# BEAMRobotics/beam_slam

Hardware: AMD Instinct MI355X
Metric: LM iterations/sec + ms/graph-solve, 200KF x 50k-landmark VIO window (higher is better)
Workload: dtype f64; 1 GPU; C2: 200-keyframe x 50000-landmark VIO window; n_obs=400690, n_imu_factors=199, solver_options=vio.yaml:7-17 (<= 10 iterations, tolerances 1.5e-7), max_solver_time lifted, parallelism=single GPU, n_ranks_seen=1

## Files before the change

beam_slam_amd/csrc/band_plan.h:

```cpp
#pragma once
#include <cstdint>
#include <vector>

#include "bsgpu_internal.h"

namespace bsg {

__host__ __device__ inline bool band_record(int b, int e, const int* cam_pose, int* cmin, int4* rec) {
  *cmin = -1;
  *rec = make_int4(0, 0, -1, -1);
  if (e - b < 2 || e - b > kBandCams) return false;
  int lo = cam_pose[b], hi = cam_pose[b];
  for (int f = b + 1; f < e; ++f) { lo = cam_pose[f] < lo ? cam_pose[f] : lo; hi = cam_pose[f] > hi ? cam_pose[f] : hi; }
  if (hi - lo >= kBandCams) return false;
  unsigned m = 0;
  uint64_t inv = ~(uint64_t)0;
  for (int f = b; f < e; ++f) {
    const int sl = cam_pose[f] - lo;
    const unsigned bit = 1u << sl;
    if (m & bit) return false;
    m |= bit;
    inv = (inv & ~((uint64_t)15 << (4 * sl))) | ((uint64_t)(f - b) << (4 * sl));
  }
  *cmin = lo;
  *rec = make_int4(b, (int)(m | ((unsigned)(hi - lo + 1) << 16) | ((unsigned)(e - b) << 24)), (int)(uint32_t)inv, (int)(uint32_t)(inv >> 32));
  return true;
}

inline void band_classify_host(int nl, const int* lm_start, const int* cam_pose, std::vector<int>& cmin, std::vector<int>& mask, std::vector<int4>& rec) {
  cmin.assign(nl, -1); mask.assign(nl, 0);
  rec.assign(nl, make_int4(0, 0, -1, -1));
  for (int l = 0; l < nl; ++l)
    if (band_record(lm_start[l], lm_start[l + 1], cam_pose, &cmin[l], &rec[l])) mask[l] = rec[l].y & 0xffff;
}

struct BandUnits {
  std::vector<int> lm;
  std::vector<int> unit_start, unit_cam;
  std::vector<uint32_t> adj;
};

int band_part_forced();

inline void band_units(int nl, const int* cmin, const int* mask, int ncp, BandUnits& out) {
  out.lm.clear(); out.unit_start.clear(); out.unit_cam.clear();
  const size_t nc = (size_t)(ncp > 0 ? ncp : 1);
  out.adj.assign(nc, 0);
  const size_t nkey = nc * 16;
  std::vector<int> start(nkey + 1, 0);
  auto span_of = [&](int l) { int top = 0; for (unsigned m = (unsigned)mask[l]; m; m >>= 1) ++top; return top; };
  auto key_of = [&](int l) { return (size_t)cmin[l] * 16 + (size_t)(kBandCams - span_of(l)); };
  int n = 0;
  for (int l = 0; l < nl; ++l) if (cmin[l] >= 0) { start[key_of(l) + 1]++; ++n; }
  out.unit_start.push_back(0);
  if (!n) return;
  for (size_t k = 0; k < nkey; ++k) start[k + 1] += start[k];
  out.lm.resize(n);
  for (int l = 0; l < nl; ++l) if (cmin[l] >= 0) out.lm[start[key_of(l)]++] = l;
  out.unit_start.clear();
  int part = band_part_forced();
  if (part <= 0) part = n / 128 > 64 ? n / 128 : 64;
  std::vector<std::vector<unsigned>> seen(nc);
  int i = 0;
  while (i < n) {
    const int k0 = cmin[out.lm[i]];
    int j = i;
    while (j < n && cmin[out.lm[j]] == k0) {
      const unsigned m = (unsigned)mask[out.lm[j]];
      bool have = false;
      for (unsigned s : seen[k0]) if (s == m) { have = true; break; }
      if (!have) {
        seen[k0].push_back(m);
        for (int a = 0; a < kBandCams; ++a)
          if ((m >> a) & 1u) out.adj[k0 + a] |= (m >> a);
      }
      ++j;
    }
    const int parts = (j - i + part - 1) / part;
    for (int p = 0; p < parts; ++p) { out.unit_start.push_back(i + (int)((int64_t)(j - i) * p / parts)); out.unit_cam.push_back(k0); }
    i = j;
  }
  out.unit_start.push_back(n);
}

}
```

beam_slam_amd/csrc/bsgpu_finalize.cpp:

```cpp
#include <atomic>

#include "bsgpu_ctx.h"
#include "bsgpu_env.h"
#include "band_plan.h"
#include "dim_order.h"

namespace bsg {

int band_part_forced() {
  return env_int("BSGPU_BAND_PART", 0);
}

namespace {
void eigen_quat_to_rot(const double* q, double* R) {
  const double tx = 2 * q[1], ty = 2 * q[2], tz = 2 * q[3];
  const double twx = tx * q[0], twy = ty * q[0], twz = tz * q[0], txx = tx * q[1], txy = ty * q[1], txz = tz * q[1];
  const double tyy = ty * q[2], tyz = tz * q[2], tzz = tz * q[3];
  R[0] = 1 - (tyy + tzz); R[1] = txy - twz; R[2] = txz + twy;
  R[3] = txy + twz; R[4] = 1 - (txx + tzz); R[5] = tyz - twx;
  R[6] = txz - twy; R[7] = tyz + twx; R[8] = 1 - (txx + tyy);
}

}

int finalize(bsgpu_ctx* c) {
  if (c->finalized) return BSGPU_OK;
  const bool timing = env_timing();
  auto t_prev = std::chrono::steady_clock::now();
  auto lap = [&](const char* what) {
    if (!timing) return;
    const auto now = std::chrono::steady_clock::now();
    fprintf(stderr, "[bsgpu finalize] %-28s %8.2f ms\n", what, std::chrono::duration<double, std::milli>(now - t_prev).count());
    t_prev = now;
  };
  c->free_device();
  HIPCHK(c, hipSetDevice(c->device));
  lap("free previous");
  const int nb = c->nb;
  if (nb <= 0) return fail(c, BSGPU_ERR_INVALID, "no parameter blocks");
  std::vector<int> lm_use(nb, 0), other_use(nb, 0), rho_use(nb, 0);
  for (int t = 0; t < BSGPU_F_NUM_TYPES; ++t) {
    const HostGroup& g = c->groups[t];
    const TypeInfo& ti = kTypes[t];
    if (t == BSGPU_F_REPROJ && c->mirror0.active && !c->mirror0.materialized) {
      const SlotMirror& m = c->mirror0;
      const size_t ns = std::max({m.use_q.size(), m.use_p.size(), m.use_l.size()});
// ... 256 lines not shown
      cp_keys.erase(std::unique(cp_keys.begin(), cp_keys.end()), cp_keys.end());
    }
    const int k = (int)cp_keys.size();
    std::vector<int> cp_tq, cp_tp, cp_first(nb, -1);
    for (int i = 0; i < k; ++i) {
      const int bq = (int)(cp_keys[i] >> 32), bp = (int)(cp_keys[i] & 0xffffffffu);
      cp_tq.push_back(c->toff[bq]); cp_tp.push_back(c->toff[bp]);
      if (cp_first[bq] < 0) cp_first[bq] = i;
    }
    auto cp_of = [&](int bq, int bp) {
      int i = cp_first[bq];
      while ((int)(cp_keys[i] & 0xffffffffu) != bp) ++i;
      return i;
    };
    V.n_cam_pose = k;
    int n_elim = 0;
    for (int i = 0; i < nv; ++i) {
      const VF& e = vf[i];
      fac[i] = make_int4(e.xq, e.xp, e.xl, meta_pack(e.meta_cam, e.loss, e.flags));
      pix[i] = make_double2(e.u, e.v);
      w[i] = e.w;
      cam_pose[i] = cp_of(e.bq, e.bp);
      lm_of[i] = e.lm;
      c->vis_src[i] = e.src;
      if (e.lm >= 0) { lm_start[e.lm + 1]++; n_elim++; }
    }
    for (int l = 0; l < nl; ++l) lm_start[l + 1] += lm_start[l];
    V.n_elim = n_elim;
    lap("camera-pose ids");
    std::vector<int> b_cmin(nl, -1), b_mask(nl, 0);
    std::vector<int4> b_rec;
    if (band_on && nl > 0) band_classify_host(nl, lm_start.data(), cam_pose.data(), b_cmin, b_mask, b_rec);
    BandUnits bu;
    band_units(nl, b_cmin.data(), b_mask.data(), V.n_cam_pose, bu);
    std::vector<int4> b_lm(bu.lm.size());
    for (size_t i = 0; i < bu.lm.size(); ++i) b_lm[i] = b_rec[bu.lm[i]];
    V.n_band_lm = (int)bu.lm.size(); V.n_band_units = (int)bu.unit_cam.size();
    lap("band landmarks");
    const uint64_t ncp = (uint64_t)std::max(1, V.n_cam_pose);
    std::vector<int> seg_ci, seg_cj, seg_start, ent_fa, ent_fb;
    if (ncp * ncp <= (uint64_t)8 << 20 && !sort_entries) {
      std::vector<int> start(ncp * ncp + 1, 0);
      for (int l = 0; l < nl; ++l) {
        if (b_cmin[l] >= 0) continue;
        for (int a = lm_start[l]; a < lm_start[l + 1]; ++a) {
          const uint64_t ra = (uint64_t)cam_pose[a] * ncp;
          for (int b = lm_start[l]; b < lm_start[l + 1]; ++b) if (cam_pose[a] <= cam_pose[b]) start[ra + cam_pose[b] + 1]++;
        }
      }
      for (int f = n_elim; f < nv; ++f) start[(uint64_t)cam_pose[f] * ncp + cam_pose[f] + 1]++;
      for (size_t i = 0; i < ncp * ncp; ++i) start[i + 1] += start[i];
      const size_t n_ent = (size_t)start[ncp * ncp];
      ent_fa.resize(n_ent); ent_fb.resize(n_ent);
      lap("count pair entries");
      const int chunk = pair_chunk(n_ent);
      for (uint64_t key = 0; key < ncp * ncp; ++key)
        for (int p0 = start[key]; p0 < start[key + 1]; p0 += chunk) { seg_ci.push_back((int)(key / ncp)); seg_cj.push_back((int)(key % ncp)); seg_start.push_back(p0); }
      std::vector<int> pos(start.begin(), start.end() - 1);
      for (int l = 0; l < nl; ++l) {
        if (b_cmin[l] >= 0) continue;
        for (int a = lm_start[l]; a < lm_start[l + 1]; ++a) {
          const uint64_t ra = (uint64_t)cam_pose[a] * ncp;
          for (int b = lm_start[l]; b < lm_start[l + 1]; ++b)
            if (cam_pose[a] <= cam_pose[b]) { const int p = pos[ra + cam_pose[b]]++; ent_fa[p] = a; ent_fb[p] = b; }
        }
      }
      for (int f = n_elim; f < nv; ++f) { const int p = pos[(uint64_t)cam_pose[f] * ncp + cam_pose[f]]++; ent_fa[p] = f; ent_fb[p] = f; }
      lap("fill pair entries");
    } else {
      struct Ent { uint64_t key; int fa, fb; };
// ... 74 lines not shown
      cb.seg_cp = c->upload(sg_cp); cb.seg_start = c->upload(sg_start); cb.seg_fac = c->upload(by_cp);
      const int re[2] = {cb.tq, cb.tp};
      for (int a = 0; a < 2; ++a) {
        for (int b = 0; b < 2; ++b) touch(re[a], re[b]);
        for (int i = 0; i < k; ++i) { touch(cp_tq[i], re[a]); touch(cp_tp[i], re[a]); }
      }
    }
  }
    return BSGPU_OK;
  };
  bool flattened_on_device = false;
  {
    const bool force_dev = env_flatten_is("device"), force_host = env_flatten_is("host");
    const HostGroup& g0 = c->groups[BSGPU_F_REPROJ];
    SlotMirror& mir = c->mirror0;
    const bool resident = mir.active && !mir.materialized && mir.dev_valid;
    if (!force_host && c->groups[BSGPU_F_REPROJ_ONLINE_CALIB].n == 0 && g0.n > 0 && (force_dev || g0.n >= kDeviceFlattenMin)) {
      bool ok = true;
      if (mir.active && !mir.materialized && !resident) { const int rc_m = materialize_mirror(c); if (rc_m != BSGPU_OK) return rc_m; }
      if (resident) { for (const auto& u : mir.loss_use) if (u.rows > 0 && ok) { get_loss(u.kind, u.a); ok = losses.size() <= 8; } }
      else for (int f = 0; f < g0.n && ok; ++f) { get_loss(g0.loss_kind[f], g0.loss_a[f]); ok = losses.size() <= 8; }
      if (ok) {
        std::vector<int> bx(c->off.begin(), c->off.end());
        std::vector<unsigned char> bc(c->is_const.begin(), c->is_const.end());
        const int* d_bx = c->upload(bx); const int* d_bt = c->upload(c->toff);
        const unsigned char* d_bc = c->upload(bc); const int* d_bl = c->upload(lm_index);
        const int T = (c->n_pose + 63) / 64;
        bool all_const = false;
        FlattenSegsHost segs_host;
        auto dalloc = [&](size_t bytes) -> void* { return c->alloc<unsigned char>(bytes); };
        const FlattenResident res = {mir.d_idx, mir.d_consts, mir.d_lk, mir.d_la, mir.d_s2b};
        const int st = flatten_visual_device(c->stream, dalloc, g0.n, g0.idx.data(), g0.consts.data(), g0.loss_kind.data(), g0.loss_a.data(),
                                             losses, nb, d_bx, d_bt, d_bc, d_bl, nl, T, c->vis, &c->d_vis_src, c->tile_adj, &all_const,
                                             resident ? &res : nullptr, bg.nbk ? &segs_host : nullptr, band_on);
        if (st < 0) return fail(c, BSGPU_ERR_DEVICE, "device error while flattening the reprojection factors");
        if (st == 0) {
          flattened_on_device = true;
          if (bg.nbk)
            for (size_t sgi = 0; sgi < segs_host.seg_ci.size(); ++sgi) {
              const int i = segs_host.seg_ci[sgi], j = segs_host.seg_cj[sgi];
              const int ri[2] = {segs_host.cp_tq[i], segs_host.cp_tp[i]}, rj[2] = {segs_host.cp_tq[j], segs_host.cp_tp[j]};
              for (int a = 0; a < 2; ++a) for (int b = 0; b < 2; ++b) if (ri[a] >= 0 && rj[b] >= 0) bg.add(ri[a], rj[b]);
            }
          if (all_const) { c->any_inactive = true; c->vis_any_inactive = true; }
          if (c->vis.n_cam_pose >= (1 << 20)) return fail(c, BSGPU_ERR_UNSUPPORTED, "too many camera poses");
        } else {
          c->vis = Visual();
        }
      }
    }
  }
  if (flattened_on_device) lap("flatten on device");
  else { const int rc_host = host_visual(); if (rc_host != BSGPU_OK) return rc_host; }
  Visual& V = c->vis;
  {
    const int nv = V.n;
    V.r = c->alloc<double2>(nv); V.J = c->alloc<double>((size_t)nv * (kJAStride + 6)); V.JB = V.J ? V.J + (size_t)nv * kJAStride : nullptr; V.CR = c->alloc<double>((size_t)nv * 8);
    V.Linv = c->alloc<double>((size_t)std::max(1, nl) * kLmRec); V.z = V.Linv ? V.Linv + 6 : nullptr;
    V.n_cost_part = (nv + 255) / 256;
    V.cost_part = c->alloc<double>(V.n_cost_part);
    V.cost_part_cand = c->alloc<double>(V.n_cost_part);
    V.mcc_part = c->alloc<double>(std::max(1, backsub_mcc_groups(V)));
    if (!V.J || !V.CR || !V.r) return fail(c, BSGPU_ERR_DEVICE, "out of device memory (visual tables)");
    if (c->calib.on) {
      c->calib.E = c->alloc<double>((size_t)std::max(1, nv) * 12); c->calib.Et = c->alloc<double>((size_t)std::max(1, nv) * 12);
      c->calib.part = c->alloc<double>((size_t)std::max(1, calib_border_blocks(V)) * kCalibPartStride);
      if (!c->calib.E || !c->calib.Et || !c->calib.part) return fail(c, BSGPU_ERR_DEVICE, "out of device memory (extrinsic border tables)");
// ... 868 lines not shown
```

beam_slam_amd/csrc/bsgpu_internal.h:

```cpp
#pragma once
#include <hip/hip_runtime.h>
#include <stdint.h>

#include <functional>
#include <cstring>
#include <vector>

#include "dense_plan.h"

struct bsgpu_options;

namespace bsg {

struct DevCamera {
  double fx, fy, cx, cy;
  double R[9];
  double t[3];
};
struct DevLoss {
  int kind;
  int pad;
  double a;
};

// ... 429 lines not shown
                               int bridge_gap, double min_excitation, int apply_scale, double scale_min, double scale_max, double rank_tol,
                               double* gravity, double* bg, double* scale, double* excitation, int* gyro_rank, double* velocity,
                               double* q_out, double* p_out, double* v_out, int* status, int* own, double* fs, double* ps);
void launch_triangulate(hipStream_t s, int n_tracks, const int* track_start, const int2* pose_off, const double2* pix, const double* x,
                        const DevCamera& cam, bool truncate, double max_dist, double max_reproj, double* points, int* status);
constexpr int kLocOutStride = 45;
void launch_localize(hipStream_t s, int n_frames, const int* obs_start, const double2* pix, const double* pts, const int* pt_off,
                     const double* x, const DevCamera* cams, const int* cam_of, const double* pose_in, int loss_kind, double loss_a,
                     double sqrt_info, int truncate, int min_points, int width, int height, const bsgpu_options& opt, double* out,
                     int* out_i);
constexpr int kRansacOutInts = 8;
void launch_essential_ransac(hipStream_t s, int n_sets, const int* match_start, const double2* px_prev, const double2* px_cur,
                             const double* K, double prob, double threshold_px, int max_iters, uint64_t seed, unsigned char* mask,
                             double* out_E, int* out_i);
constexpr int kP3pOutDoubles = 19;
constexpr int kP3pOutInts = 6;
void launch_absolute_pose_ransac(hipStream_t s, int n_frames, const int* obs_start, const double2* pix, const double* pts,
                                 const DevCamera* cams, const int* cam_of, double prob, double threshold_px, int max_iters, uint64_t seed,
                                 int truncate, unsigned char* mask, double* out_d, int* out_i);
constexpr int kRelposeOutDoubles = 27;
constexpr int kRelposeOutInts = 11;
void launch_relative_pose_ransac(hipStream_t s, int n_sets, const int* match_start, const double2* pix_first, const double2* pix_last,
                                 const DevCamera* cams, const int* cam_of, double prob, double threshold_px, int max_iters, uint64_t seed,
                                 int truncate, double validate_px, double min_inlier_ratio, unsigned char* mask, unsigned char* valid_mask,
                                 double* points, double* out_d, int* out_i);
struct FlattenResident { const int* idx; const double* consts; const int* loss_kind; const double* loss_a; const int* slot_map; };
struct FlattenSegsHost { std::vector<int> seg_ci, seg_cj, cp_tq, cp_tp; };
void launch_patch_factor_rows(hipStream_t s, int n_ch, const int* rows, const int* idx4, const double* consts3, const int* lk, const double* la,
                              int* dst_idx, double* dst_consts, int* dst_lk, double* dst_la);
int flatten_visual_device(hipStream_t s, const std::function<void*(size_t)>& dalloc, int n, const int* h_idx, const double* h_consts,
                          const int* h_loss_kind, const double* h_loss_a, const std::vector<DevLoss>& losses, int nb, const int* d_blk_xoff,
                          const int* d_blk_toff, const unsigned char* d_blk_const, const int* d_blk_lm, int nl, int T, Visual& V,
                          int** d_vis_src, std::vector<unsigned char>& tile_adj, bool* any_all_const, const FlattenResident* res = nullptr,
                          FlattenSegsHost* segs_out = nullptr, bool band_enabled = true);
int chol_vinv_stride();
void chol_prepare();
void launch_bsr_assemble(hipStream_t s, const SmallGroup& g, const int* slots, double* val);
void launch_bsr_assemble_seg(hipStream_t s, const SmallGroup* groups_dev, int n_seg, const int* seg_start, const int* seg_slot, const int* seg_row,
                             const int2* contrib, double* val, double* rhs, double* grad, double* hdiag);
void launch_bsr_finish_diag(hipStream_t s, int nbr, const int* diag_slot, const int* pair_slot, double* val, const double* hdiag, double radius,
                            int compute_scale, int compute_dcl, int jacobi, double lm_lo, double lm_hi, double* scale,
                            double* dcl, double* Minv);
int pcg_spmv_grid(int nbr);
struct PcgPersistDev {
  int G = 0, max_cols = 0;
  int paired = 0;
  const int *wg_row = nullptr, *wg_colptr = nullptr, *wg_cols = nullptr, *lcol = nullptr;
  unsigned long long* slots = nullptr;
  int* abort_w = nullptr;
  double* zg = nullptr;
  size_t sync_bytes = 0;
  int n_coarse = 0;
  const int4* co = nullptr;
  double centre[3] = {0.0, 0.0, 0.0};
  double *W = nullptr, *E = nullptr, *Einv = nullptr;
  unsigned* counter = nullptr;
};
size_t pcg_coarse_scratch_doubles(int nbr);
void launch_pcg_coarse(hipStream_t s, const PcgPersistDev& P, int nbr, const int* row_ptr, const int* col, const double* val, const double* x);
size_t pcg_persistent_lds(int max_cols);
size_t pcg_persistent_lds_limit();
int pcg_persistent_max_rows();
size_t pcg_persistent_slot_words(int G);
size_t pcg_persistent_z_words(int nbr);
bool launch_pcg_persistent(hipStream_t s, const PcgPersistDev& P, int nbr, const int* row_ptr, const double* val, const double* Minv, const double* b,
                           double* x, double* zg, double* sc, double tol2, int max_it);
void launch_pcg_init(hipStream_t s, int nbr, const double* b, const double* Minv, double* x, double* r, double* z, double* p0, double* p1,
// ... 50 lines not shown
```

beam_slam_amd/csrc/k_flatten.hip:

```cpp
#include <string.h>

#include <cstring>

#include <rocprim/rocprim.hpp>

#include <cstdint>
#include <functional>
#include <vector>

#include "bsgpu_device.h"
#include "band_plan.h"

namespace bsg {

namespace {

__global__ void fl_prep_kernel(int n, const int* __restrict__ idx , const double* __restrict__ consts ,
                               const int* __restrict__ loss_kind, const double* __restrict__ loss_a, int n_loss,
                               const int* __restrict__ tab_kind, const double* __restrict__ tab_a, const int* __restrict__ blk_xoff,
                               const unsigned char* __restrict__ blk_const, const int* __restrict__ blk_lm, int nl,
                               unsigned* __restrict__ key, int4* __restrict__ fac, double2* __restrict__ pix, double* __restrict__ w,
                               int* __restrict__ lm_of, int* __restrict__ bq_of, int* __restrict__ used_q, int* __restrict__ p_of_q,
                               int* __restrict__ flags_out ,
                               const int* __restrict__ slot_map ) {
  const int f = blockIdx.x * 256 + threadIdx.x;
  if (f >= n) return;
  const int4 row = reinterpret_cast<const int4*>(idx)[f];
  const int bq = slot_map ? slot_map[row.x] : row.x, bp = slot_map ? slot_map[row.y] : row.y, bl = slot_map ? slot_map[row.z] : row.z;
  const int cam = row.w;
  const int lm = blk_lm[bl];
  const int cq = blk_const[bq], cp = blk_const[bp], cl = blk_const[bl];
  if (lm < 0 && !cl) flags_out[0] = 1;
  const int fl = (cq ? kFlagQConst : 0) | (cp ? kFlagPConst : 0) | (cl ? kFlagLConst : 0);
  if (fl == 7) flags_out[1] = 1;
  int kind = loss_kind[f];
  double a = loss_a[f];
  if (kind == BSGPU_LOSS_TRIVIAL) a = 1.0;
  int lid = -1;
  for (int i = 0; i < n_loss; ++i) if (tab_kind[i] == kind && tab_a[i] == a) { lid = i; break; }
  if (lid < 0) { flags_out[0] = 1; lid = 0; }
  key[f] = (unsigned)(lm < 0 ? nl : lm);
  fac[f] = make_int4(blk_xoff[bq], blk_xoff[bp], blk_xoff[bl], meta_pack(cam, lid, fl));
  pix[f] = make_double2(consts[3 * f], consts[3 * f + 1]);
  w[f] = consts[3 * f + 2];
// ... 7 lines not shown
__global__ void fl_cp_kernel(int nb, const int* __restrict__ used_q, const int* __restrict__ cp_of_q, const int* __restrict__ p_of_q,
                             const int* __restrict__ blk_toff, int* __restrict__ cp_tq, int* __restrict__ cp_tp) {
  const int b = blockIdx.x * 256 + threadIdx.x;
  if (b >= nb || !used_q[b]) return;
  cp_tq[cp_of_q[b]] = blk_toff[b];
  cp_tp[cp_of_q[b]] = blk_toff[p_of_q[b]];
}

__global__ void fl_gather_kernel(int n, const int* __restrict__ order, const int4* __restrict__ fac_in, const double2* __restrict__ pix_in,
                                 const double* __restrict__ w_in, const int* __restrict__ lm_in, const int* __restrict__ bq_in,
                                 const int* __restrict__ cp_of_q, int4* __restrict__ fac, double2* __restrict__ pix,
                                 double* __restrict__ w, int* __restrict__ lm_of, int* __restrict__ cam_pose, int* __restrict__ src,
                                 int* __restrict__ lm_cnt) {
  const int i = blockIdx.x * 256 + threadIdx.x;
  if (i >= n) return;
  const int f = order[i];
  fac[i] = fac_in[f]; pix[i] = pix_in[f]; w[i] = w_in[f];
  const int lm = lm_in[f];
  lm_of[i] = lm;
  cam_pose[i] = cp_of_q[bq_in[f]];
  src[i] = f;
  if (lm >= 0) atomicAdd(&lm_cnt[lm], 1);
}

__global__ void fl_band_kernel(int nl, const int* __restrict__ lm_start, const int* __restrict__ cam_pose, int enabled, int* __restrict__ cmin,
                               int* __restrict__ mask, int4* __restrict__ rec) {
  const int l = blockIdx.x * 256 + threadIdx.x;
  if (l >= nl) return;
  int cm = -1;
  int4 rc = make_int4(0, 0, -1, -1);
  if (enabled) band_record(lm_start[l], lm_start[l + 1], cam_pose, &cm, &rc);
  cmin[l] = cm; mask[l] = cm >= 0 ? (rc.y & 0xffff) : 0; rec[l] = rc;
}
__global__ void fl_band_gather_kernel(int n, const int* __restrict__ order, const int4* __restrict__ rec, int4* __restrict__ out) {
  const int i = blockIdx.x * 256 + threadIdx.x;
  if (i < n) out[i] = rec[order[i]];
}

__global__ void fl_pair_count_kernel(int nl, const int* __restrict__ lm_start, const int* __restrict__ cam_pose, const int* __restrict__ cmin,
                                     int* __restrict__ cnt) {
  const int l = blockIdx.x * 256 + threadIdx.x;
  if (l >= nl) return;
  int n = 0;
  if (cmin[l] < 0)
    for (int a = lm_start[l]; a < lm_start[l + 1]; ++a)
      for (int b = lm_start[l]; b < lm_start[l + 1]; ++b) n += cam_pose[a] <= cam_pose[b];
  cnt[l] = n;
}
__global__ void fl_pair_gen_kernel(int nl, const int* __restrict__ lm_start, const int* __restrict__ cam_pose, const int* __restrict__ cmin,
                                   const int* __restrict__ off, unsigned long long ncp, unsigned long long* __restrict__ key,
                                   unsigned long long* __restrict__ val) {
  const int l = blockIdx.x * 256 + threadIdx.x;
  if (l >= nl || cmin[l] >= 0) return;
  int o = off[l];
  for (int a = lm_start[l]; a < lm_start[l + 1]; ++a)
    for (int b = lm_start[l]; b < lm_start[l + 1]; ++b)
      if (cam_pose[a] <= cam_pose[b]) {
        key[o] = (unsigned long long)cam_pose[a] * ncp + (unsigned long long)cam_pose[b];
        val[o] = ((unsigned long long)(unsigned)a << 32) | (unsigned)b;
        ++o;
      }
}
__global__ void fl_pair_tail_kernel(int n_elim, int n, const int* __restrict__ cam_pose, unsigned long long ncp, int base,
                                    unsigned long long* __restrict__ key, unsigned long long* __restrict__ val) {
  const int i = n_elim + blockIdx.x * 256 + threadIdx.x;
  if (i >= n) return;
  const int o = base + (i - n_elim);
  key[o] = (unsigned long long)cam_pose[i] * ncp + (unsigned long long)cam_pose[i];
  val[o] = ((unsigned long long)(unsigned)i << 32) | (unsigned)i;
// ... 21 lines not shown
  const int ri[2] = {cp_tq[ci], cp_tp[ci]}, rj[2] = {cp_tq[cj], cp_tp[cj]};
  for (int a = 0; a < 2; ++a) for (int b = 0; b < 2; ++b) {
    if (ri[a] < 0 || rj[b] < 0) continue;
    for (int x = ri[a]; x < ri[a] + 3; x += 2) for (int y = rj[b]; y < rj[b] + 3; y += 2) {
      tile_adj[(size_t)(x / 64) * T + y / 64] = 1; tile_adj[(size_t)(y / 64) * T + x / 64] = 1;
    }
  }
}

__global__ void fl_patch_kernel(int n_ch, const int* __restrict__ rows, const int4* __restrict__ idx4, const double* __restrict__ consts3,
                                const int* __restrict__ lk, const double* __restrict__ la, int4* __restrict__ dst_idx,
                                double* __restrict__ dst_consts, int* __restrict__ dst_lk, double* __restrict__ dst_la) {
  const int i = blockIdx.x * 256 + threadIdx.x;
  if (i >= n_ch) return;
  const size_t r = (size_t)rows[i];
  dst_idx[r] = idx4[i];
  dst_consts[3 * r] = consts3[3 * i]; dst_consts[3 * r + 1] = consts3[3 * i + 1]; dst_consts[3 * r + 2] = consts3[3 * i + 2];
  dst_lk[r] = lk[i]; dst_la[r] = la[i];
}

}

void launch_patch_factor_rows(hipStream_t s, int n_ch, const int* rows, const int* idx4, const double* consts3, const int* lk, const double* la,
                              int* dst_idx, double* dst_consts, int* dst_lk, double* dst_la) {
  if (n_ch <= 0) return;
  hipLaunchKernelGGL(fl_patch_kernel, dim3((n_ch + 255) / 256), dim3(256), 0, s, n_ch, rows, reinterpret_cast<const int4*>(idx4), consts3, lk, la,
                     reinterpret_cast<int4*>(dst_idx), dst_consts, dst_lk, dst_la);
}

int flatten_visual_device(hipStream_t s, const std::function<void*(size_t)>& dalloc, int n, const int* h_idx, const double* h_consts,
                          const int* h_loss_kind, const double* h_loss_a, const std::vector<DevLoss>& losses, int nb, const int* d_blk_xoff,
                          const int* d_blk_toff, const unsigned char* d_blk_const, const int* d_blk_lm, int nl, int T, Visual& V,
                          int** d_vis_src, std::vector<unsigned char>& tile_adj, bool* any_all_const, const FlattenResident* res,
                          FlattenSegsHost* segs_out, bool band_enabled) {
  auto A = [&](size_t bytes) { return dalloc(bytes ? bytes : 8); };
#define FL_CHK(x) do { if ((x) != hipSuccess) { (void)hipGetLastError(); return -1; } } while (0)
  const int g256 = (n + 255) / 256;
  int* d_idx = res ? const_cast<int*>(res->idx) : (int*)A(sizeof(int) * 4 * (size_t)n);
  double* d_consts = res ? const_cast<double*>(res->consts) : (double*)A(sizeof(double) * 3 * (size_t)n);
  int* d_lk = res ? const_cast<int*>(res->loss_kind) : (int*)A(sizeof(int) * (size_t)n);
  double* d_la = res ? const_cast<double*>(res->loss_a) : (double*)A(sizeof(double) * (size_t)n);
  const int n_loss = (int)losses.size();
  std::vector<int> tk(n_loss); std::vector<double> ta(n_loss);
  for (int i = 0; i < n_loss; ++i) { tk[i] = losses[i].kind; ta[i] = losses[i].a; }
  int* d_tk = (int*)A(sizeof(int) * n_loss); double* d_ta = (double*)A(sizeof(double) * n_loss);
  unsigned *d_key = (unsigned*)A(sizeof(unsigned) * (size_t)n), *d_key2 = (unsigned*)A(sizeof(unsigned) * (size_t)n);
  int4* d_fac0 = (int4*)A(sizeof(int4) * (size_t)n); double2* d_pix0 = (double2*)A(sizeof(double2) * (size_t)n);
  double* d_w0 = (double*)A(sizeof(double) * (size_t)n);
  int *d_lm0 = (int*)A(sizeof(int) * (size_t)n), *d_bq0 = (int*)A(sizeof(int) * (size_t)n),
      *d_order = (int*)A(sizeof(int) * (size_t)n);
  int *d_used = (int*)A(sizeof(int) * ((size_t)nb + 1)), *d_pofq = (int*)A(sizeof(int) * (size_t)nb), *d_cpofq = (int*)A(sizeof(int) * ((size_t)nb + 1));
  int* d_flags = (int*)A(sizeof(int) * 4);
  if (!d_idx || !d_consts || !d_lk || !d_la || !d_key || !d_key2 || !d_fac0 || !d_pix0 || !d_w0 || !d_lm0 || !d_bq0 || !d_order ||
      !d_used || !d_pofq || !d_cpofq || !d_flags || !d_tk || !d_ta) return -1;
  if (!res) {
    FL_CHK(hipMemcpyAsync(d_idx, h_idx, sizeof(int) * 4 * (size_t)n, hipMemcpyHostToDevice, s));
    FL_CHK(hipMemcpyAsync(d_consts, h_consts, sizeof(double) * 3 * (size_t)n, hipMemcpyHostToDevice, s));
    FL_CHK(hipMemcpyAsync(d_lk, h_loss_kind, sizeof(int) * (size_t)n, hipMemcpyHostToDevice, s));
    FL_CHK(hipMemcpyAsync(d_la, h_loss_a, sizeof(double) * (size_t)n, hipMemcpyHostToDevice, s));
  }
  FL_CHK(hipMemcpyAsync(d_tk, tk.data(), sizeof(int) * n_loss, hipMemcpyHostToDevice, s));
  FL_CHK(hipMemcpyAsync(d_ta, ta.data(), sizeof(double) * n_loss, hipMemcpyHostToDevice, s));
  FL_CHK(hipMemsetAsync(d_used, 0, sizeof(int) * ((size_t)nb + 1), s));
  FL_CHK(hipMemsetAsync(d_pofq, 0xff, sizeof(int) * (size_t)nb, s));
  FL_CHK(hipMemsetAsync(d_flags, 0, sizeof(int) * 4, s));
  hipLaunchKernelGGL(fl_prep_kernel, dim3(g256), dim3(256), 0, s, n, d_idx, d_consts, d_lk, d_la, n_loss, d_tk, d_ta, d_blk_xoff, d_blk_const,
                     d_blk_lm, nl, d_key, d_fac0, d_pix0, d_w0, d_lm0, d_bq0, d_used, d_pofq, d_flags, res ? res->slot_map : nullptr);
// ... 19 lines not shown
  V.fac = (int4*)A(sizeof(int4) * (size_t)n); V.pix = (double2*)A(sizeof(double2) * (size_t)n); V.w = (double*)A(sizeof(double) * (size_t)n);
  V.lm_of = (int*)A(sizeof(int) * (size_t)n); V.cam_pose = (int*)A(sizeof(int) * (size_t)n);
  *d_vis_src = (int*)A(sizeof(int) * (size_t)n);
  int* d_lmcnt = (int*)A(sizeof(int) * ((size_t)nl + 1));
  V.lm_start = (int*)A(sizeof(int) * ((size_t)nl + 1));
  int *d_pcnt = (int*)A(sizeof(int) * ((size_t)nl + 1)), *d_poff = (int*)A(sizeof(int) * ((size_t)nl + 1));
  if (!V.fac || !V.pix || !V.w || !V.lm_of || !V.cam_pose || !*d_vis_src || !d_lmcnt || !V.lm_start || !d_pcnt || !d_poff) return -1;
  FL_CHK(hipMemsetAsync(d_lmcnt, 0, sizeof(int) * ((size_t)nl + 1), s));
  FL_CHK(hipMemsetAsync(d_pcnt, 0, sizeof(int) * ((size_t)nl + 1), s));
  hipLaunchKernelGGL(fl_gather_kernel, dim3(g256), dim3(256), 0, s, n, d_order, d_fac0, d_pix0, d_w0, d_lm0, d_bq0, d_cpofq, V.fac, V.pix, V.w,
                     V.lm_of, V.cam_pose, *d_vis_src, d_lmcnt);
  size_t need2 = 0;
  FL_CHK(rocprim::exclusive_scan(nullptr, need2, d_lmcnt, V.lm_start, 0, (size_t)nl + 1, rocprim::plus<int>(), s));
  void* d_tmp2 = need2 > tmp_bytes ? A(need2) : d_tmp;
  size_t tmp2_bytes = need2 > tmp_bytes ? need2 : tmp_bytes;
  if (!d_tmp2) return -1;
  FL_CHK(rocprim::exclusive_scan(d_tmp2, tmp2_bytes, d_lmcnt, V.lm_start, 0, (size_t)nl + 1, rocprim::plus<int>(), s));
  int *d_bcmin = (int*)A(sizeof(int) * ((size_t)nl + 1)), *d_bmask = (int*)A(sizeof(int) * ((size_t)nl + 1));
  int4* d_brec = (int4*)A(sizeof(int4) * ((size_t)nl + 1));
  if (!d_bcmin || !d_bmask || !d_brec) return -1;
  std::vector<int> h_bcmin(nl), h_bmask(nl);
  if (nl > 0) {
    hipLaunchKernelGGL(fl_band_kernel, dim3((nl + 255) / 256), dim3(256), 0, s, nl, V.lm_start, V.cam_pose, band_enabled ? 1 : 0, d_bcmin, d_bmask, d_brec);
    hipLaunchKernelGGL(fl_pair_count_kernel, dim3((nl + 255) / 256), dim3(256), 0, s, nl, V.lm_start, V.cam_pose, d_bcmin, d_pcnt);
    FL_CHK(hipMemcpyAsync(h_bcmin.data(), d_bcmin, sizeof(int) * (size_t)nl, hipMemcpyDeviceToHost, s));
    FL_CHK(hipMemcpyAsync(h_bmask.data(), d_bmask, sizeof(int) * (size_t)nl, hipMemcpyDeviceToHost, s));
  }
  FL_CHK(rocprim::exclusive_scan(d_tmp2, tmp2_bytes, d_pcnt, d_poff, 0, (size_t)nl + 1, rocprim::plus<int>(), s));
  int h_nelim = 0, h_npairs = 0;
  FL_CHK(hipMemcpyAsync(&h_nelim, V.lm_start + nl, sizeof(int), hipMemcpyDeviceToHost, s));
  FL_CHK(hipMemcpyAsync(&h_npairs, d_poff + nl, sizeof(int), hipMemcpyDeviceToHost, s));
  FL_CHK(hipStreamSynchronize(s));
  BandUnits bu;
  band_units(nl, h_bcmin.data(), h_bmask.data(), h_ncp, bu);
  V.n_band_lm = (int)bu.lm.size(); V.n_band_units = (int)bu.unit_cam.size();
  V.band_lm = (int4*)A(sizeof(int4) * bu.lm.size()); V.band_unit_start = (int*)A(sizeof(int) * bu.unit_start.size());
  V.band_unit_cam = (int*)A(sizeof(int) * bu.unit_cam.size());
  int* d_border = (int*)A(sizeof(int) * bu.lm.size());
  if (!V.band_lm || !V.band_unit_start || !V.band_unit_cam || !d_border) return -1;
  if (!bu.lm.empty()) {
    FL_CHK(hipMemcpyAsync(d_border, bu.lm.data(), sizeof(int) * bu.lm.size(), hipMemcpyHostToDevice, s));
    hipLaunchKernelGGL(fl_band_gather_kernel, dim3(((int)bu.lm.size() + 255) / 256), dim3(256), 0, s, (int)bu.lm.size(), d_border, d_brec, V.band_lm);
    V.band_lm_id = d_border;
  }
  FL_CHK(hipMemcpyAsync(V.band_unit_start, bu.unit_start.data(), sizeof(int) * bu.unit_start.size(), hipMemcpyHostToDevice, s));
  if (!bu.unit_cam.empty()) FL_CHK(hipMemcpyAsync(V.band_unit_cam, bu.unit_cam.data(), sizeof(int) * bu.unit_cam.size(), hipMemcpyHostToDevice, s));
  V.n_elim = h_nelim;
  const int n_ent = h_npairs + (n - h_nelim);
  V.n_ent = n_ent;
  const unsigned long long ncp = (unsigned long long)(h_ncp > 0 ? h_ncp : 1);
  unsigned long long *d_ek = (unsigned long long*)A(8 * (size_t)n_ent), *d_ev = (unsigned long long*)A(8 * (size_t)n_ent),
                     *d_ek2 = (unsigned long long*)A(8 * (size_t)n_ent), *d_ev2 = (unsigned long long*)A(8 * (size_t)n_ent);
  V.ent_fa = (int*)A(sizeof(int) * (size_t)n_ent); V.ent_fb = (int*)A(sizeof(int) * (size_t)n_ent);
  int *d_runidx = (int*)A(sizeof(int) * (size_t)n_ent), *d_runstart = (int*)A(sizeof(int) * (size_t)n_ent);
  unsigned char* d_segflag = (unsigned char*)A((size_t)n_ent);
  int* d_segsel = (int*)A(sizeof(int) * ((size_t)n_ent + 1));
  int* d_nseg = (int*)A(sizeof(int) * 2);
  if (!d_ek || !d_ev || !d_ek2 || !d_ev2 || !V.ent_fa || !V.ent_fb || !d_runidx || !d_runstart || !d_segflag || !d_segsel || !d_nseg) return -1;
  if (nl > 0 && h_npairs > 0) hipLaunchKernelGGL(fl_pair_gen_kernel, dim3((nl + 255) / 256), dim3(256), 0, s, nl, V.lm_start, V.cam_pose, d_bcmin, d_poff, ncp, d_ek, d_ev);
  if (n > h_nelim) hipLaunchKernelGGL(fl_pair_tail_kernel, dim3((n - h_nelim + 255) / 256), dim3(256), 0, s, h_nelim, n, V.cam_pose, ncp, h_npairs, d_ek, d_ev);
  int kbits = 1;
  while (kbits < 64 && (ncp * ncp) >> kbits) ++kbits;
  size_t need3 = 0, need4 = 0, need5 = 0;
  if (n_ent > 0) {
    FL_CHK(rocprim::radix_sort_pairs(nullptr, need3, d_ek, d_ek2, d_ev, d_ev2, (size_t)n_ent, 0, kbits, s));
    FL_CHK(rocprim::inclusive_scan(nullptr, need4, d_runidx, d_runstart, (size_t)n_ent, rocprim::maximum<int>(), s));
    FL_CHK(rocprim::select(nullptr, need5, rocprim::counting_iterator<int>(0), d_segflag, d_segsel, d_nseg, (size_t)n_ent, s));
    size_t need345 = need3 > need4 ? need3 : need4;
    if (need5 > need345) need345 = need5;
    void* d_tmp3 = need345 > tmp2_bytes ? A(need345) : d_tmp2;
    size_t tmp3_bytes = need345 > tmp2_bytes ? need345 : tmp2_bytes;
    if (!d_tmp3) return -1;
    FL_CHK(rocprim::radix_sort_pairs(d_tmp3, tmp3_bytes, d_ek, d_ek2, d_ev, d_ev2, (size_t)n_ent, 0, kbits, s));
    const int ge = (n_ent + 255) / 256;
    hipLaunchKernelGGL(fl_split_kernel, dim3(ge), dim3(256), 0, s, n_ent, d_ek2, d_ev2, V.ent_fa, V.ent_fb, d_runidx);
// ... 56 lines not shown
```

Before: 3799 LM iterations/s.

## Pack band landmark units by modelled cost to fit the CU budget

Replaces the fixed per-camera partition of banded landmarks with a cost-model-driven packing. Landmarks from adjacent starting cameras can now be merged into one unit, with their records rebased by a shift, and a binary search on a per-unit cost cap keeps the unit count within a budget taken from the CU count minus a reserve for other factor kernels. The aim is to balance the band Schur-complement work across CUs and avoid one long straggler unit per iteration. It adds host-side planning cost at finalize and a hand-tuned cost model that could misjudge the real kernel cost.

After: 3795 LM iterations/s. No clear change (-0.1%).

```diff
diff --git a/beam_slam_amd/csrc/band_plan.h b/beam_slam_amd/csrc/band_plan.h
--- a/beam_slam_amd/csrc/band_plan.h
+++ b/beam_slam_amd/csrc/band_plan.h
@@ -34,21 +34,75 @@
     if (band_record(lm_start[l], lm_start[l + 1], cam_pose, &cmin[l], &rec[l])) mask[l] = rec[l].y & 0xffff;
 }
 
+__host__ __device__ inline int4 band_rebase(int4 rec, int d) {
+  if (d <= 0) return rec;
+  const uint64_t inv = (uint64_t)(uint32_t)rec.z | ((uint64_t)(uint32_t)rec.w << 32);
+  const uint64_t out = (inv << (4 * d)) | (((uint64_t)1 << (4 * d)) - 1);
+  const unsigned y = (unsigned)rec.y;
+  const unsigned mask = (y & 0xffffu) << d, span = ((y >> 16) & 0xffu) + (unsigned)d;
+  return make_int4(rec.x, (int)(mask | (span << 16) | (y & 0xff000000u)), (int)(uint32_t)out, (int)(uint32_t)(out >> 32));
+}
+
 struct BandUnits {
   std::vector<int> lm;
+  std::vector<int> shift;
   std::vector<int> unit_start, unit_cam;
   std::vector<uint32_t> adj;
+  int longest_subs = 0, longest_cost = 0;
 };
 
 int band_part_forced();
 
-inline void band_units(int nl, const int* cmin, const int* mask, int ncp, BandUnits& out) {
-  out.lm.clear(); out.unit_start.clear(); out.unit_cam.clear();
+constexpr int kBandCostSub = 26, kBandCostPass = 5, kBandCostFlush = 3;
+constexpr int kBandRiderUs10 = 40, kBandUnitUs10 = 320;
+inline int band_unit_budget(int n_cu, int riders) {
+  if (n_cu <= 0) return 0;
+  int reserve = (int)(((int64_t)(riders > 0 ? riders : 0) * kBandRiderUs10 + kBandUnitUs10 - 1) / kBandUnitUs10);
+  if (reserve < 8) reserve = 8;
+  if (reserve > n_cu / 4) reserve = n_cu / 4;
+  return n_cu - reserve > 1 ? n_cu - reserve : 1;
+}
+
+inline int band_tile_rows(int span) { return (6 * span + 15) >> 4; }
+inline int band_unit_cost(const int* hist, int n) {
+  if (n <= 0) return 0;
+  int cost = 0, at = 0, e = kBandCams, left = hist[kBandCams], first = 1;
+  while (at < n) {
+    while (left == 0 && e > 0) left = hist[--e];
+    const int T = band_tile_rows(e);
+    if (first) { cost += kBandCostFlush * (T * (T + 1) / 2); first = 0; }
+    cost += kBandCostSub + kBandCostPass * ((T * (T + 1) / 2 + 3) / 4);
+    int take = 32;
+    while (take > 0 && at < n) {
+      while (left == 0 && e > 0) left = hist[--e];
+      const int k = left < take ? left : take;
+      left -= k; take -= k; at += k;
+    }
+  }
+  return cost;
+}
+
+inline void band_units_stats(BandUnits& out, const int* cmin, const int* mask) {
+  for (size_t u = 0; u + 1 < out.unit_start.size(); ++u) {
+    int hist[kBandCams + 1] = {0};
+    const int b = out.unit_start[u], e = out.unit_start[u + 1];
+    for (int i = b; i < e; ++i) { int top = 0; for (unsigned m = (unsigned)mask[out.lm[i]]; m; m >>= 1) ++top; hist[cmin[out.lm[i]] - out.unit_cam[u] + top]++; }
+    const int c = band_unit_cost(hist, e - b);
+    if (c > out.longest_cost) out.longest_cost = c;
+    if ((e - b + 31) / 32 > out.longest_subs) out.longest_subs = (e - b + 31) / 32;
+  }
+}
+
+inline void band_units(int nl, const int* cmin, const int* mask, int ncp, BandUnits& out, int max_units) {
+  out.lm.clear(); out.shift.clear(); out.unit_start.clear(); out.unit_cam.clear();
+  out.longest_subs = out.longest_cost = 0;
   const size_t nc = (size_t)(ncp > 0 ? ncp : 1);
   out.adj.assign(nc, 0);
   const size_t nkey = nc * 16;
   std::vector<int> start(nkey + 1, 0);
-  auto span_of = [&](int l) { int top = 0; for (unsigned m = (unsigned)mask[l]; m; m >>= 1) ++top; return top; };
+  std::vector<unsigned char> span(nl > 0 ? nl : 0, 0);
+  for (int l = 0; l < nl; ++l) if (cmin[l] >= 0) { int top = 0; for (unsigned m = (unsigned)mask[l]; m; m >>= 1) ++top; span[l] = (unsigned char)top; }
+  auto span_of = [&](int l) { return (int)span[l]; };
   auto key_of = [&](int l) { return (size_t)cmin[l] * 16 + (size_t)(kBandCams - span_of(l)); };
   int n = 0;
   for (int l = 0; l < nl; ++l) if (cmin[l] >= 0) { start[key_of(l) + 1]++; ++n; }
@@ -58,29 +112,116 @@
   out.lm.resize(n);
   for (int l = 0; l < nl; ++l) if (cmin[l] >= 0) out.lm[start[key_of(l)]++] = l;
   out.unit_start.clear();
-  int part = band_part_forced();
-  if (part <= 0) part = n / 128 > 64 ? n / 128 : 64;
-  std::vector<std::vector<unsigned>> seen(nc);
-  int i = 0;
-  while (i < n) {
-    const int k0 = cmin[out.lm[i]];
-    int j = i;
-    while (j < n && cmin[out.lm[j]] == k0) {
-      const unsigned m = (unsigned)mask[out.lm[j]];
-      bool have = false;
-      for (unsigned s : seen[k0]) if (s == m) { have = true; break; }
-      if (!have) {
-        seen[k0].push_back(m);
+  out.shift.assign(n, 0);
+  {
+    std::vector<unsigned> seen;
+    int i = 0;
+    while (i < n) {
+      const int k0 = cmin[out.lm[i]];
+      seen.clear();
+      for (; i < n && cmin[out.lm[i]] == k0; ++i) {
+        const unsigned m = (unsigned)mask[out.lm[i]];
+        bool have = false;
+        for (unsigned s : seen) if (s == m) { have = true; break; }
+        if (have) continue;
+        seen.push_back(m);
         for (int a = 0; a < kBandCams; ++a)
           if ((m >> a) & 1u) out.adj[k0 + a] |= (m >> a);
       }
-      ++j;
-    }
-    const int parts = (j - i + part - 1) / part;
-    for (int p = 0; p < parts; ++p) { out.unit_start.push_back(i + (int)((int64_t)(j - i) * p / parts)); out.unit_cam.push_back(k0); }
-    i = j;
-  }
+    }
+  }
+  const int forced = band_part_forced();
+  if (forced < 0 || (forced == 0 && max_units <= 0)) {
+    const int part = n / 128 > 64 ? n / 128 : 64;
+    int i = 0;
+    while (i < n) {
+      const int k0 = cmin[out.lm[i]];
+      int j = i;
+      while (j < n && cmin[out.lm[j]] == k0) ++j;
+      const int parts = (j - i + part - 1) / part;
+      for (int p = 0; p < parts; ++p) { out.unit_start.push_back(i + (int)((int64_t)(j - i) * p / parts)); out.unit_cam.push_back(k0); }
+      i = j;
+    }
+    out.unit_start.push_back(n);
+    band_units_stats(out, cmin, mask);
+    return;
+  }
+  struct Run { int cam, span, beg, cnt; };
+  std::vector<Run> runs;
+  for (size_t k = 0; k < nkey; ++k) {
+    const int b = k ? start[k - 1] : 0, e = start[k];
+    if (e > b) runs.push_back({(int)(k / 16), kBandCams - (int)(k % 16), b, e - b});
+  }
+  const int kNoCap = 1 << 30;
+  auto pass = [&](int cap_n, int cap_cost, bool emit) {
+    int units = 0, hist[kBandCams + 1] = {0}, cnt = 0, base = -1, ubeg = 0;
+    auto close = [&](int end) {
+      if (cnt == 0) return;
+      ++units;
+      if (emit) { out.unit_start.push_back(ubeg); out.unit_cam.push_back(base); }
+      for (int e = 0; e <= kBandCams; ++e) hist[e] = 0;
+      cnt = 0; ubeg = end;
+    };
+    for (const Run& r : runs) {
+      int done = 0;
+      while (done < r.cnt) {
+        if (cnt > 0 && r.cam - base + r.span > kBandCams) close(r.beg + done);
+        if (cnt == 0) base = r.cam;
+        const int e = r.cam - base + r.span;
+        auto fits = [&](int k) {
+          if (cnt + k > cap_n) return false;
+          if (cap_cost == kNoCap) return true;
+          if (kBandCostFlush * 15 + ((cnt + k + 31) / 32) * (kBandCostSub + 4 * kBandCostPass) <= cap_cost) return true;
+          hist[e] += k;
+          const int c = band_unit_cost(hist, cnt + k);
+          hist[e] -= k;
+          return c <= cap_cost;
+        };
+        int k = r.cnt - done;
+        if (!fits(k)) {
+          int lo = 0, hi = k;
+          while (hi - lo > 1) { const int mid = (lo + hi) / 2; if (fits(mid)) lo = mid; else hi = mid; }
+          k = lo;
+          if (k == 0 && cnt == 0) k = 1;
+        }
+        hist[e] += k; cnt += k; done += k;
+        if (done < r.cnt) close(r.beg + done);
+      }
+    }
+    close(n);
+    return units;
+  };
+  int cap_n = kNoCap, cap_cost = kNoCap;
+  if (forced > 0) cap_n = forced;
+  else {
+    int umax = max_units < n / 64 ? max_units : n / 64;
+    if (umax < 1) umax = 1;
+    const int subs = ((n + umax - 1) / umax + 31) / 32;
+    int want = (n + 32 * subs - 1) / (32 * subs);
+    const int floor_units = pass(kNoCap, kNoCap, false);
+    if (want < floor_units) want = floor_units;
+    const int share = (n + want - 1) / want;
+    int lo = kBandCostSub, hi = kBandCostFlush * 15 + ((share + 31) / 32) * (kBandCostSub + 4 * kBandCostPass);
+    while (hi < (1 << 28) && pass(kNoCap, hi, false) > want) { lo = hi; hi *= 2; }
+    while (hi - lo > 1) { const int mid = lo + (hi - lo) / 2; if (pass(kNoCap, mid, false) <= want) hi = mid; else lo = mid; }
+    cap_cost = hi;
+  }
+  (void)pass(cap_n, cap_cost, true);
   out.unit_start.push_back(n);
-}
-
-}
+  std::vector<int> tmp, tsh;
+  for (size_t u = 0; u + 1 < out.unit_start.size(); ++u) {
+    const int b = out.unit_start[u], e = out.unit_start[u + 1], base = out.unit_cam[u];
+    int at[kBandCams + 2] = {0};
+    for (int i = b; i < e; ++i) at[kBandCams - (cmin[out.lm[i]] - base + span_of(out.lm[i])) + 1]++;
+    for (int k = 0; k <= kBandCams; ++k) at[k + 1] += at[k];
+    tmp.resize(e - b); tsh.resize(e - b);
+    for (int i = b; i < e; ++i) {
+      const int d = cmin[out.lm[i]] - base, p = at[kBandCams - (d + span_of(out.lm[i]))]++;
+      tmp[p] = out.lm[i]; tsh[p] = d;
+    }
+    for (int i = b; i < e; ++i) { out.lm[i] = tmp[i - b]; out.shift[i] = tsh[i - b]; }
+  }
+  band_units_stats(out, cmin, mask);
+}
+
+}
diff --git a/beam_slam_amd/csrc/bsgpu_finalize.cpp b/beam_slam_amd/csrc/bsgpu_finalize.cpp
--- a/beam_slam_amd/csrc/bsgpu_finalize.cpp
+++ b/beam_slam_amd/csrc/bsgpu_finalize.cpp
@@ -12,6 +12,21 @@
 }
 
 namespace {
+int band_max_units(const bsgpu_ctx* c) {
+  static std::atomic<int> n_cu_of[64];
+  const int dev = c->device >= 0 && c->device < 64 ? c->device : 0;
+  int n_cu = n_cu_of[dev].load(std::memory_order_relaxed);
+  if (n_cu == 0) {
+    hipDeviceProp_t pr;
+    n_cu = hipGetDeviceProperties(&pr, c->device) == hipSuccess && pr.multiProcessorCount > 0 ? pr.multiProcessorCount : 256;
+    n_cu_of[dev].store(n_cu, std::memory_order_relaxed);
+  }
+  int riders = 0;
+  for (int t = BSGPU_F_IMU_DELTA; t < BSGPU_F_NUM_TYPES; ++t)
+    if (t != BSGPU_F_IDP_REPROJ && t != BSGPU_F_IDP_REPROJ_UNARY) riders += c->groups[t].n;
+  return band_unit_budget(n_cu, riders);
+}
+
 void eigen_quat_to_rot(const double* q, double* R) {
   const double tx = 2 * q[1], ty = 2 * q[2], tz = 2 * q[3];
   const double twx = tx * q[0], twy = ty * q[0], twz = tz * q[0], txx = tx * q[1], txy = ty * q[1], txz = tz * q[1];
@@ -334,10 +349,11 @@
     std::vector<int4> b_rec;
     if (band_on && nl > 0) band_classify_host(nl, lm_start.data(), cam_pose.data(), b_cmin, b_mask, b_rec);
     BandUnits bu;
-    band_units(nl, b_cmin.data(), b_mask.data(), V.n_cam_pose, bu);
+    band_units(nl, b_cmin.data(), b_mask.data(), V.n_cam_pose, bu, band_max_units(c));
     std::vector<int4> b_lm(bu.lm.size());
-    for (size_t i = 0; i < bu.lm.size(); ++i) b_lm[i] = b_rec[bu.lm[i]];
+    for (size_t i = 0; i < bu.lm.size(); ++i) b_lm[i] = band_rebase(b_rec[bu.lm[i]], bu.shift[i]);
     V.n_band_lm = (int)bu.lm.size(); V.n_band_units = (int)bu.unit_cam.size();
+    if (timing && V.n_band_units > 0) fprintf(stderr, "[bsgpu finalize] band units %d (budget %d), longest: %d sub-batches, modelled %.1f us\n", V.n_band_units, band_max_units(c), bu.longest_subs, 0.1 * bu.longest_cost);
     lap("band landmarks");
     const uint64_t ncp = (uint64_t)std::max(1, V.n_cam_pose);
     std::vector<int> seg_ci, seg_cj, seg_start, ent_fa, ent_fb;
@@ -478,7 +494,7 @@
         const FlattenResident res = {mir.d_idx, mir.d_consts, mir.d_lk, mir.d_la, mir.d_s2b};
         const int st = flatten_visual_device(c->stream, dalloc, g0.n, g0.idx.data(), g0.consts.data(), g0.loss_kind.data(), g0.loss_a.data(),
                                              losses, nb, d_bx, d_bt, d_bc, d_bl, nl, T, c->vis, &c->d_vis_src, c->tile_adj, &all_const,
-                                             resident ? &res : nullptr, bg.nbk ? &segs_host : nullptr, band_on);
+                                             resident ? &res : nullptr, bg.nbk ? &segs_host : nullptr, band_on, band_max_units(c));
         if (st < 0) return fail(c, BSGPU_ERR_DEVICE, "device error while flattening the reprojection factors");
         if (st == 0) {
           flattened_on_device = true;
diff --git a/beam_slam_amd/csrc/bsgpu_internal.h b/beam_slam_amd/csrc/bsgpu_internal.h
--- a/beam_slam_amd/csrc/bsgpu_internal.h
+++ b/beam_slam_amd/csrc/bsgpu_internal.h
@@ -485,7 +485,7 @@
                           const int* h_loss_kind, const double* h_loss_a, const std::vector<DevLoss>& losses, int nb, const int* d_blk_xoff,
                           const int* d_blk_toff, const unsigned char* d_blk_const, const int* d_blk_lm, int nl, int T, Visual& V,
                           int** d_vis_src, std::vector<unsigned char>& tile_adj, bool* any_all_const, const FlattenResident* res = nullptr,
-                          FlattenSegsHost* segs_out = nullptr, bool band_enabled = true);
+                          FlattenSegsHost* segs_out = nullptr, bool band_enabled = true, int band_max_units = 0);
 int chol_vinv_stride();
 void chol_prepare();
 void launch_bsr_assemble(hipStream_t s, const SmallGroup& g, const int* slots, double* val);
diff --git a/beam_slam_amd/csrc/k_flatten.hip b/beam_slam_amd/csrc/k_flatten.hip
--- a/beam_slam_amd/csrc/k_flatten.hip
+++ b/beam_slam_amd/csrc/k_flatten.hip
@@ -5,11 +5,13 @@
 #include <rocprim/rocprim.hpp>
 
 #include <cstdint>
+#include <cstdio>
 #include <functional>
 #include <vector>
 
 #include "bsgpu_device.h"
 #include "band_plan.h"
+#include "bsgpu_env.h"
 
 namespace bsg {
 
@@ -83,9 +85,9 @@
   if (enabled) band_record(lm_start[l], lm_start[l + 1], cam_pose, &cm, &rc);
   cmin[l] = cm; mask[l] = cm >= 0 ? (rc.y & 0xffff) : 0; rec[l] = rc;
 }
-__global__ void fl_band_gather_kernel(int n, const int* __restrict__ order, const int4* __restrict__ rec, int4* __restrict__ out) {
-  const int i = blockIdx.x * 256 + threadIdx.x;
-  if (i < n) out[i] = rec[order[i]];
+__global__ void fl_band_gather_kernel(int n, const int* __restrict__ order, const int* __restrict__ shift, const int4* __restrict__ rec, int4* __restrict__ out) {
+  const int i = blockIdx.x * 256 + threadIdx.x;
+  if (i < n) out[i] = band_rebase(rec[order[i]], shift[i]);
 }
 
 __global__ void fl_pair_count_kernel(int nl, const int* __restrict__ lm_start, const int* __restrict__ cam_pose, const int* __restrict__ cmin,
@@ -173,7 +175,7 @@
                           const int* h_loss_kind, const double* h_loss_a, const std::vector<DevLoss>& losses, int nb, const int* d_blk_xoff,
                           const int* d_blk_toff, const unsigned char* d_blk_const, const int* d_blk_lm, int nl, int T, Visual& V,
                           int** d_vis_src, std::vector<unsigned char>& tile_adj, bool* any_all_const, const FlattenResident* res,
-                          FlattenSegsHost* segs_out, bool band_enabled) {
+                          FlattenSegsHost* segs_out, bool band_enabled, int band_max_units) {
   auto A = [&](size_t bytes) { return dalloc(bytes ? bytes : 8); };
 #define FL_CHK(x) do { if ((x) != hipSuccess) { (void)hipGetLastError(); return -1; } } while (0)
   const int g256 = (n + 255) / 256;
@@ -259,15 +261,18 @@
   FL_CHK(hipMemcpyAsync(&h_npairs, d_poff + nl, sizeof(int), hipMemcpyDeviceToHost, s));
   FL_CHK(hipStreamSynchronize(s));
   BandUnits bu;
-  band_units(nl, h_bcmin.data(), h_bmask.data(), h_ncp, bu);
+  band_units(nl, h_bcmin.data(), h_bmask.data(), h_ncp, bu, band_max_units);
   V.n_band_lm = (int)bu.lm.size(); V.n_band_units = (int)bu.unit_cam.size();
+  if (env_timing() && V.n_band_units > 0) fprintf(stderr, "[bsgpu finalize] band units %d (budget %d), longest: %d sub-batches, modelled %.1f us\n", V.n_band_units, band_max_units, bu.longest_subs, 0.1 * bu.longest_cost);
   V.band_lm = (int4*)A(sizeof(int4) * bu.lm.size()); V.band_unit_start = (int*)A(sizeof(int) * bu.unit_start.size());
   V.band_unit_cam = (int*)A(sizeof(int) * bu.unit_cam.size());
   int* d_border = (int*)A(sizeof(int) * bu.lm.size());
-  if (!V.band_lm || !V.band_unit_start || !V.band_unit_cam || !d_border) return -1;
+  int* d_bshift = (int*)A(sizeof(int) * bu.lm.size());
+  if (!V.band_lm || !V.band_unit_start || !V.band_unit_cam || !d_border || !d_bshift) return -1;
   if (!bu.lm.empty()) {
     FL_CHK(hipMemcpyAsync(d_border, bu.lm.data(), sizeof(int) * bu.lm.size(), hipMemcpyHostToDevice, s));
-    hipLaunchKernelGGL(fl_band_gather_kernel, dim3(((int)bu.lm.size() + 255) / 256), dim3(256), 0, s, (int)bu.lm.size(), d_border, d_brec, V.band_lm);
+    FL_CHK(hipMemcpyAsync(d_bshift, bu.shift.data(), sizeof(int) * bu.shift.size(), hipMemcpyHostToDevice, s));
+    hipLaunchKernelGGL(fl_band_gather_kernel, dim3(((int)bu.lm.size() + 255) / 256), dim3(256), 0, s, (int)bu.lm.size(), d_border, d_bshift, d_brec, V.band_lm);
     V.band_lm_id = d_border;
   }
   FL_CHK(hipMemcpyAsync(V.band_unit_start, bu.unit_start.data(), sizeof(int) * bu.unit_start.size(), hipMemcpyHostToDevice, s));
```
